# lighttransport/pbrlab

Hardware: AMD Instinct MI355X
Metric: Msamples/s (paths x spp / s), 1920x1080 Cornell-box-Suzanne render (higher is better)
Workload: dtype f32

## Files before the change

### pbrlab_amd/csrc/bvh_build.cpp

```cpp
#include <math.h>
#include <stdlib.h>
#include <string.h>

#include <algorithm>
#include <atomic>
#include <deque>
#include <functional>
#include <future>
#include <limits>
#include <thread>

#include "host_scene.h"
#include "qquant.h"

namespace pb {
namespace {

#ifndef PB_SAH_BINS
#define PB_SAH_BINS 48
#endif
constexpr int kBins = PB_SAH_BINS;
#ifndef PB_SAH_SWEEP
#define PB_SAH_SWEEP 256
#endif
#ifndef PB_MAX_LEAF_CURVES
#define PB_MAX_LEAF_CURVES PB_MAX_LEAF
#endif
constexpr float kTraversalCost = 1.0f;
constexpr float kPrimCost = 1.5f;

struct Box {
  float lo[3], hi[3];
  void reset() {
    for (int a = 0; a < 3; a++) lo[a] = std::numeric_limits<float>::infinity(), hi[a] = -lo[a];
  }
  void grow(const float* l, const float* h) {
    for (int a = 0; a < 3; a++) {
      lo[a] = std::min(lo[a], l[a]);
      hi[a] = std::max(hi[a], h[a]);
    }
  }
  void grow(const Box& b) { grow(b.lo, b.hi); }
  float area() const {
    float dx = hi[0] - lo[0], dy = hi[1] - lo[1], dz = hi[2] - lo[2];
    if (!(dx >= 0 && dy >= 0 && dz >= 0)) return 0.f;
    return 2.f * (dx * dy + dy * dz + dz * dx);
  }
};

struct TNode {
  Box box;
  int32_t left = -1, right = -1;
  uint32_t first = 0, count = 0;
  uint8_t kind = 0;
  uint32_t depth = 1;
};

struct Builder {
// ... 82 lines not shown
        }
        float rarea[kBins];
        uint32_t rcnt[kBins];
        Box acc;
        acc.reset();
        uint32_t n = 0;
        for (int k = kBins - 1; k > 0; k--) {
          acc.grow(bb[k]);
          n += bc[k];
          rarea[k] = acc.area();
          rcnt[k] = n;
        }
        acc.reset();
        n = 0;
        for (int k = 0; k < kBins - 1; k++) {
          acc.grow(bb[k]);
          n += bc[k];
          if (n == 0 || rcnt[k + 1] == 0) continue;
          float cost = acc.area() * (float)n + rarea[k + 1] * (float)rcnt[k + 1];
          if (cost < best_cost) best_cost = cost, best_axis = a, best_bin = k;
        }
      }
      if (best_axis >= 0) {
        float scale = (float)kBins / (cbox.hi[best_axis] - cbox.lo[best_axis]);
        float base = cbox.lo[best_axis];
        mid = (uint32_t)(std::partition(order.begin() + first, order.begin() + first + count,
                                        [&](uint32_t g) {
                                          int k = std::min(kBins - 1, std::max(0, (int)((cen[3 * g + best_axis] - base) * scale)));
                                          return k <= best_bin;
                                        }) -
                         order.begin());
      }
      if (mid == first || mid == first + count) {
        int a = 0;
        for (int c = 1; c < 3; c++)
          if (cbox.hi[c] - cbox.lo[c] > cbox.hi[a] - cbox.lo[a]) a = c;
        mid = first + count / 2;
        std::nth_element(order.begin() + first, order.begin() + mid, order.begin() + first + count,
                         [&](uint32_t x, uint32_t y) { return cen[3 * x + a] < cen[3 * y + a] || (cen[3 * x + a] == cen[3 * y + a] && x < y); });
      }
    }
    int32_t l = build(pool, first, mid - first, depth + 1);
    int32_t r = build(pool, mid, first + count - mid, depth + 1);
    pool.nodes[id].left = l;
    pool.nodes[id].right = r;
    return id;
  }
};

uint32_t leaf_ref(const TNode& n) {
  return kLeafBit | (n.kind ? kCurveBit : 0u) | (n.first << 3) | (n.count - 1u);
}

}

void build_bvh(const std::vector<float>& lo, const std::vector<float>& hi, const std::vector<uint8_t>& kinds,
               FlatBvh* out) {
  out->nodes.clear();
  out->slot_gid.clear();
  out->depth = 0;
  uint32_t n = (uint32_t)kinds.size();
  if (n == 0) return;
  Builder b;
  b.lo = lo.data(), b.hi = hi.data(), b.kinds = kinds.data();
  b.cen.resize(3 * (size_t)n);
  b.order.resize(n);
  for (uint32_t g = 0; g < n; g++) {
    for (int a = 0; a < 3; a++) b.cen[3 * g + a] = 0.5f * (lo[3 * g + a] + hi[3 * g + a]);
    b.order[g] = g;
  }
  Builder::Pool pool;
  pool.nodes.reserve(2 * (size_t)n / 2 + 16);
  int32_t root = b.build(pool, 0, n, 1);

  const std::vector<TNode>& T = pool.nodes;
  const float kNaN3[3] = {std::numeric_limits<float>::quiet_NaN(), std::numeric_limits<float>::quiet_NaN(),
                          std::numeric_limits<float>::quiet_NaN()};
  std::vector<BvhNode>& N = out->nodes;
  uint32_t depth = 0;
  if (T[root].left < 0) {
    BvhNode nd;
    memset(&nd, 0, sizeof(nd));
    nd.set_box(0, T[root].box.lo, T[root].box.hi);
    nd.set_box(1, kNaN3, kNaN3);
    nd.c0 = leaf_ref(T[root]);
    nd.c1 = kEmptyChild;
    N.push_back(nd);
    depth = 1;
  } else {
    struct Item {
      int32_t t;
      uint32_t out;
    };
    std::deque<Item> work;
    N.emplace_back();
    work.push_back({root, 0});
    while (!work.empty()) {
      Item it;
      if (N.size() < (size_t)kTopNodes) it = work.front(), work.pop_front();
      else it = work.back(), work.pop_back();
      const TNode& t = T[it.t];
      depth = std::max(depth, t.depth);
      BvhNode nd;
      memset(&nd, 0, sizeof(nd));
      const TNode &l = T[t.left], &r = T[t.right];
      nd.set_box(0, l.box.lo, l.box.hi);
      nd.set_box(1, r.box.lo, r.box.hi);
      if (l.left < 0) {
        nd.c0 = leaf_ref(l);
      } else {
        nd.c0 = (uint32_t)N.size();
        N.emplace_back();
        work.push_back({t.left, nd.c0});
      }
      if (r.left < 0) {
        nd.c1 = leaf_ref(r);
      } else {
        nd.c1 = (uint32_t)N.size();
        N.emplace_back();
        work.push_back({t.right, nd.c1});
      }
      N[it.out] = nd;
    }
  }
  out->slot_gid = b.order;
  out->depth = depth;
}


uint32_t qtree_stack_need(const std::vector<QNode>& N) {
  if (N.empty()) return 0;
  std::vector<uint32_t> need(N.size(), 0);
  std::vector<uint8_t> state(N.size(), 0);
  std::vector<uint32_t> todo{0u};
  while (!todo.empty()) {
    const uint32_t i = todo.back();
    const QNode& nd = N[i];
    if (state[i] == 0) {
      state[i] = 1;
      for (int k = 0; k < 4; k++)
        if (!(nd.c[k] & kLeafBit) && nd.c[k] < N.size() && state[nd.c[k]] == 0) todo.push_back(nd.c[k]);
      continue;
    }
    todo.pop_back();
    if (state[i] == 2) continue;
    state[i] = 2;
    uint32_t nc = 0, deepest = 0;
    for (int k = 0; k < 4; k++) {
      if (nd.c[k] == kEmptyChild) continue;
      nc++;
      if (!(nd.c[k] & kLeafBit) && nd.c[k] < N.size()) deepest = std::max(deepest, need[nd.c[k]]);
    }
    need[i] = (nc ? nc - 1u : 0u) + deepest;
  }
  return need[0];
}

uint32_t build_qtree(const std::vector<BvhNode>& N2, const std::function<uint32_t(uint32_t)>& map_leaf, std::vector<QNode>* out) {
  out->clear();
  if (N2.empty()) return 0;
  struct V {
    float lo[3], hi[3];
    int32_t l = -1, r = -1;
    uint32_t ref = 0;
    uint32_t prims = 0;
  };
  std::vector<V> T;
  T.reserve(N2.size() * 2 + 1);
  {
    struct Todo {
      uint32_t node2;
      int32_t v;
    };
    std::vector<Todo> todo;
    T.emplace_back();
    todo.push_back({0u, 0});
    while (!todo.empty()) {
      const Todo t = todo.back();
      todo.pop_back();
      const BvhNode& b = N2[t.node2];
      int32_t kids[2] = {-1, -1};
      int nk = 0;
      for (int k = 0; k < 2; k++) {
        const uint32_t ref = k ? b.c1 : b.c0;
        if (ref == kEmptyChild) continue;
        const int32_t v = (int32_t)T.size();
        T.emplace_back();
        for (int a = 0; a < 3; a++) T[v].lo[a] = b.lo[a][k], T[v].hi[a] = b.hi[a][k];
        kids[nk++] = v;
        if (ref & kLeafBit) T[v].ref = map_leaf(ref), T[v].prims = (ref & 7u) + 1u;
        else todo.push_back({ref, v});
      }
      if (nk == 2) T[t.v].l = kids[0], T[t.v].r = kids[1];
      else if (nk == 1) T[t.v].l = kids[0], T[t.v].r = -1;
    }
    for (int a = 0; a < 3; a++) {
      T[0].lo[a] = std::numeric_limits<float>::infinity(), T[0].hi[a] = -T[0].lo[a];
      for (int32_t k : {T[0].l, T[0].r})
        if (k >= 0) T[0].lo[a] = std::min(T[0].lo[a], T[k].lo[a]), T[0].hi[a] = std::max(T[0].hi[a], T[k].hi[a]);
    }
  }
  auto area = [](const V& v) {
    const float dx = v.hi[0] - v.lo[0], dy = v.hi[1] - v.lo[1], dz = v.hi[2] - v.lo[2];
    const float a = dx * dy + dy * dz + dz * dx;
    return a >= 0.f && std::isfinite(a) ? (double)a : 0.0;
  };
  constexpr double kCostNode = 1.0, kCostPrim = 1.0;
  const size_t nv = T.size();
  std::vector<double> below(nv, 0.0);
  std::vector<int32_t> choice(nv * 4, -1);
  auto qarea = [&](const V& u, const V& v) {
    double e[3];
    for (int a = 0; a < 3; a++) {
      const double ext = (double)v.hi[a] - (double)v.lo[a];
      const double st = std::max(ext / 253.0, 1e-37);
      const double ql = floor(((double)u.lo[a] - (double)v.lo[a]) / st), qh = ceil(((double)u.hi[a] - (double)v.lo[a]) / st);
      e[a] = std::max(qh - ql, 0.0) * st;
    }
    const double a = e[0] * e[1] + e[1] * e[2] + e[2] * e[0];
    return std::isfinite(a) ? a : 0.0;
  };
  for (size_t vi = nv; vi-- > 0;) {
    const V& v = T[vi];
    if (v.l < 0) continue;
    if (v.r < 0) {
      choice[vi * 4] = v.l;
      below[vi] = T[v.l].l < 0 ? area(T[v.l]) * kCostPrim * T[v.l].prims : area(T[v.l]) * kCostNode + below[v.l];
      continue;
    }
    int32_t fronts[16][4];
    int sizes[16], nf = 0;
    fronts[0][0] = v.l, fronts[0][1] = v.r, sizes[0] = 2, nf = 1;
    for (int i = 0; i < nf && nf < 16; i++) {
      if (sizes[i] >= 4) continue;
      for (int m = 0; m < sizes[i] && nf < 16; m++) {
        const V& u = T[fronts[i][m]];
        if (u.l < 0 || u.r < 0) continue;
        int32_t g[4];
        int n = 0;
        for (int j = 0; j < sizes[i]; j++) {
          if (j == m) g[n++] = u.l, g[n++] = u.r;
          else g[n++] = fronts[i][j];
        }
        std::sort(g, g + n);
        bool dup = false;
        for (int q = 0; q < nf && !dup; q++) dup = sizes[q] == n && std::equal(g, g + n, fronts[q]);
        if (dup) continue;
        std::copy(g, g + n, fronts[nf]), sizes[nf] = n, nf++;
      }
    }
    double best = 1e300;
    int bi = 0;
    for (int i = 0; i < nf; i++) {
      double c = 0.0;
      for (int m = 0; m < sizes[i]; m++) {
        const V& u = T[fronts[i][m]];
        c += u.l < 0 ? qarea(u, v) * kCostPrim * u.prims : qarea(u, v) * kCostNode + below[fronts[i][m]];
      }
      if (c < best) best = c, bi = i;
    }
    below[vi] = best;
    for (int m = 0; m < sizes[bi]; m++) choice[vi * 4 + m] = fronts[bi][m];
  }
  struct Item {
    int32_t v;
    uint32_t out;
  };
  std::deque<Item> work;
  out->emplace_back();
  work.push_back({0, 0u});
  while (!work.empty()) {
    Item it;
    if (out->size() < (size_t)kTopNodes) it = work.front(), work.pop_front();
    else it = work.back(), work.pop_back();
    int32_t fr[4];
    int n = 0;
    if (T[it.v].l < 0) {
      fr[n++] = it.v;
    } else {
      for (int m = 0; m < 4; m++)
        if (choice[(size_t)it.v * 4 + m] >= 0) fr[n++] = choice[(size_t)it.v * 4 + m];
    }
    QBox c[4];
    for (int i = 0; i < n; i++)
      for (int a = 0; a < 3; a++) c[i].lo[a] = T[fr[i]].lo[a], c[i].hi[a] = T[fr[i]].hi[a];
    QNode nd;
    if (n == 0 || !quantise_node(c, n, &nd)) {
      out->clear();
      return 0;
    }
    for (int i = 0; i < 4; i++) nd.c[i] = kEmptyChild;
    for (int i = 0; i < n; i++) {
      const V& u = T[fr[i]];
      if (u.l < 0) {
        nd.c[i] = u.ref;
      } else {
        const uint32_t id = (uint32_t)out->size();
        out->emplace_back();
        nd.c[i] = id;
        work.push_back({fr[i], id});
      }
    }
    (*out)[it.out] = nd;
  }
  return qtree_stack_need(*out);
}

void build_qlayout(const FlatBvh& bvh, const std::vector<float4>& slots, const std::vector<uint8_t>& kinds, QLayout* out) {
  static_assert(kMaxLeaf <= 2, "a leaf of the binary tree becomes one TriPair / one curve record");
  *out = QLayout();
  std::vector<float4>&qtri = out->tri, &qpts = out->pts;
  std::vector<uint32_t>& qhit = out->hit;
  const float4 zero = make_float4(0.f, 0.f, 0.f, 0.f);
  auto code = [&](uint32_t k) { return k | __builtin_bit_cast(uint32_t, slots[4 * (size_t)k + 2].w); };
  const bool tri_pairs = std::all_of(kinds.begin(), kinds.end(), [](uint8_t kd) { return kd == 0; });
  auto tri_leaf = [&](uint32_t first, uint32_t count) -> uint32_t {
// ... 113 lines not shown
```

### pbrlab_amd/csrc/commit.cpp

```cpp
#include <math.h>
#include <string.h>

#include <chrono>
#include <limits>
#include <numeric>

#include "scene_impl.h"

using namespace pb;

static_assert(sizeof(LightRec) == 80, "light record layout");

static V3 mesh_vertex(const HostMesh& m, uint32_t prim, int k) {
  const float* p = m.vertices.data() + (size_t)m.vid[prim * 3 + k] * 4;
  return V3(p[0], p[1], p[2]);
}
static V3 xf_point(const float* m, V3 v) {
  return V3(m[0] * v.x + m[4] * v.y + m[8] * v.z + m[12], m[1] * v.x + m[5] * v.y + m[9] * v.z + m[13],
            m[2] * v.x + m[6] * v.y + m[10] * v.z + m[14]);
}
static V3 world_vertex(const HostInstance& in, const HostMesh& m, uint32_t prim, int k) {
  const V3 v = mesh_vertex(m, prim, k);
  return in.identity ? v : xf_point(in.xf, v);
}
// ... 270 lines not shown
  sl[2].w = __builtin_bit_cast(float, route);
  sr.instance_id = pr.instance_id, sr.geom_id = pr.geom_id, sr.prim_id = pr.prim_id;
  return PBRHIP_OK;
}
static std::vector<BvhNode> light_boxes(const std::vector<LightHead>& heads, const std::vector<LightRec>& lrecs) {
  std::vector<BvhNode> boxes((heads.size() + 1) / 2);
  for (size_t l = 0; l < heads.size(); l++) {
    float lo3[3] = {INFINITY, INFINITY, INFINITY}, hi3[3] = {-INFINITY, -INFINITY, -INFINITY};
    for (uint32_t f = heads[l].first; f < heads[l].first + heads[l].count; f++)
      for (const float* p : {lrecs[f].p0, lrecs[f].p1, lrecs[f].p2})
        for (int a = 0; a < 3; a++) lo3[a] = std::min(lo3[a], p[a]), hi3[a] = std::max(hi3[a], p[a]);
    BvhNode& nd = boxes[l / 2];
    if (l % 2 == 0) memset(&nd, 0, sizeof(nd)), nd.set_box(1, lo3, hi3);
    nd.set_box(int(l % 2), lo3, hi3);
  }
  return boxes;
}

static double ms_since(std::chrono::steady_clock::time_point t) {
  return std::chrono::duration<double, std::milli>(std::chrono::steady_clock::now() - t).count();
}

struct CommitStage {
  std::vector<PrimRef> prims;
  std::vector<float> lo, hi, lprim_cdf;
  std::vector<uint8_t> kinds;
  FlatBvh bvh;
  std::vector<float4> slots;
  std::vector<ShadeRec> shade;
  std::vector<Material> mats;
  QLayout q;
  std::vector<LightRec> lrecs;
  std::vector<BvhNode> lboxes;
  std::vector<SssEntry> walk_entries;
};

static void stage_lights(pbrhip_scene* s, CommitStage* cs) {
  for (uint32_t i = 0; i < s->instances.size(); i++) register_lights(s, i);
  commit_lights(s);
  light_records(s, &s->light_heads, &cs->lrecs, &cs->lprim_cdf);
  cs->lboxes = light_boxes(s->light_heads, cs->lrecs);
  s->num_lrecs = (uint32_t)cs->lrecs.size();
  s->lights_transformed = std::any_of(s->lights.begin(), s->lights.end(), [&](const HostLight& L) { return !s->instances[L.instance_id].identity; });
}
static int upload_lights(pbrhip_scene* s, const CommitStage& cs) {
  HIPCHK(s->d_light_cdf.upload(s->light_cdf, s->stream));
  HIPCHK(s->d_heads.upload(s->light_heads, s->stream));
  HIPCHK(s->d_lprim_cdf.upload(cs.lprim_cdf, s->stream));
  HIPCHK(s->d_lrecs.upload(cs.lrecs, s->stream));
  HIPCHK(s->d_light_boxes.upload(cs.lboxes, s->stream));
  return PBRHIP_OK;
}

static int build_binary_tree(pbrhip_scene* s, int builder, CommitStage* cs) {
  FlatBvh& bvh = cs->bvh;
  const uint32_t np = (uint32_t)cs->prims.size();
  s->bvh_built_on_gpu = false;
  if ((builder == PBRHIP_BVH_GPU_LBVH || builder == PBRHIP_BVH_GPU_LBVH_WIDE) && np > 0) {
    HIPCHK(s->tree.reserve_nodes(TreeBufs::lbvh_nodes(np), np));
    HIPCHK(build_bvh_gpu(s->stream, cs->lo, cs->hi, cs->kinds, s->tree.d_nodes.p, &bvh.slot_gid, &bvh.depth));
    s->bvh_built_on_gpu = bvh.depth <= (uint32_t)kStackDepth;
    if (!s->bvh_built_on_gpu) {
      fprintf(stderr, "pbrhip: GPU-built BVH is %u deep (stack %d): building on the host instead\n", bvh.depth, kStackDepth);
      bvh = FlatBvh();
    }
  }
  if (!s->bvh_built_on_gpu) build_bvh(cs->lo, cs->hi, cs->kinds, &bvh);
  if (bvh.depth > (uint32_t)kStackDepth)
    return fail(PBRHIP_EOVERFLOW, "BVH depth %u exceeds the traversal stack (%d)", bvh.depth, kStackDepth);
  s->bvh_depth = bvh.depth;
  if (!s->bvh_built_on_gpu) {
    HIPCHK(s->tree.reserve_nodes((uint32_t)bvh.nodes.size(), (uint32_t)bvh.slot_gid.size()));
    if (!bvh.nodes.empty()) HIPCHK(hipMemcpyAsync(s->tree.d_nodes.p, bvh.nodes.data(), bvh.nodes.size() * sizeof(BvhNode), hipMemcpyHostToDevice, s->stream));
  }
  return PBRHIP_OK;
}

static int stage_slots_and_materials(pbrhip_scene* s, CommitStage* cs) {
  const uint32_t ns = (uint32_t)cs->bvh.slot_gid.size();
  if (ns > kHitSlotMask) return fail(PBRHIP_EINVAL, "%u traversal primitives: at most %u are supported", ns, kHitSlotMask);
  cs->slots.resize(4 * (size_t)ns), cs->shade.resize(ns);
  for (uint32_t k = 0; k < ns; k++)
    if (int rc = slot_and_shade(s, cs->prims[cs->bvh.slot_gid[k]], cs->bvh.slot_gid[k], s->light_heads, &cs->slots[4 * (size_t)k], cs->shade[k])) return rc;
  std::vector<Material>& mats = cs->mats;
  mats.resize(s->materials.size());
  s->has_hair = s->has_sss = s->has_textured = false;
  for (size_t i = 0; i < mats.size(); i++) {
    const HostMaterial& hm = s->materials[i];
    if (hm.kind == kMatPrincipled)
      for (uint32_t t : {hm.pr.base_color_tex_id, hm.pr.subsurface_color_tex_id})
        if (t != kNone && t >= s->tex_descs.size()) return fail(PBRHIP_EINVAL, "material %zu: texture id %u out of range", i, t);
    mats[i] = make_material(s->materials[i]);
    if (mats[i].textured) s->has_sss = s->has_textured = true;
    s->has_hair = s->has_hair || mats[i].kind == kMatHair;
    s->has_sss = s->has_sss || (mats[i].kind == kMatPrincipled && mats[i].bsdf.enable_subsurface);
  }
  return PBRHIP_OK;
}

static int build_wide_tree(pbrhip_scene* s, const Knobs& k, int builder, CommitStage* cs) {
  TreeBufs& t = s->tree;
  QLayout& q = cs->q;
  s->wide_built_on_gpu = false;
  if (!s->bvh_built_on_gpu && t.num_nodes && k.wide) {
    build_qlayout(cs->bvh, cs->slots, cs->kinds, &q);
    if (k.debug) fprintf(stderr, "pbrhip: commit: curve leaves of the Q tree (counted over the collapse's visits): %zu of one piece, %zu of two pieces\n", q.leaves_one, q.leaves_pair);
  }
  if (s->bvh_built_on_gpu && builder == PBRHIP_BVH_GPU_LBVH_WIDE && k.wide) {
    const bool tri_pairs = all_triangles(cs->kinds);
    QCollapse qc;
    HIPCHK(hipStreamSynchronize(s->stream));
    const auto t_start = std::chrono::steady_clock::now();
    HIPCHK(collapse_qtree_gpu(s->stream, t.d_nodes.p, t.num_slots, t.slots(), tri_pairs, [&](auto... a) { return t.alloc_wide(a...); }, &qc));
    const double ms_collapse = ms_since(t_start);
    const char* why = !qc.fits ? "a record index overflows its reference" : (!qc.quantised ? "a node cannot be quantised" : nullptr);
    if (!why) {
      q.nodes.resize(qc.nodes);
      HIPCHK(hipMemcpyAsync(q.nodes.data(), t.d_wide.p, (size_t)qc.nodes * sizeof(QNode), hipMemcpyDeviceToHost, s->stream));
      HIPCHK(hipStreamSynchronize(s->stream));
      q.stack_need = qtree_stack_need(q.nodes);
// ... 14 lines not shown
  s->wide_stack_need = q.nodes.empty() ? 0u : q.stack_need;
  return PBRHIP_OK;
}

static void accumulate_instance_bounds(std::vector<float>& ilo, std::vector<float>& ihi, size_t inst, const float* lo, const float* hi) {
  for (size_t a = 0; a < 3; a++) ilo[3 * inst + a] = std::min(ilo[3 * inst + a], lo[a]), ihi[3 * inst + a] = std::max(ihi[3 * inst + a], hi[a]);
}

static int update_walk_entries(pbrhip_scene* s, const Knobs& k, bool want, const std::vector<float>& ilo, const std::vector<float>& ihi, CommitStage* cs, double* ms) {
  cs->walk_entries.clear();
  if (want && !cs->q.nodes.empty()) {
    const auto t_entries = std::chrono::steady_clock::now();
    cs->walk_entries = build_sss_entries(cs->q.nodes, ilo, ihi, std::min(k.sss_foreign, kSssMaxForeign));
    if (ms) *ms = ms_since(t_entries);
  }
  s->num_walk_entries = (uint32_t)cs->walk_entries.size();
  if (cs->walk_entries.empty()) s->d_sss_entries.release();
  else HIPCHK(s->d_sss_entries.upload(cs->walk_entries, s->stream));
  return PBRHIP_OK;
}

void pb::bind_dscene(pbrhip_scene* s) {
  DScene& d = s->dscene;
  const TreeBufs& t = s->tree;
  d.nodes = t.d_nodes.p, d.slots = t.slots(), d.num_nodes = t.num_nodes, d.num_slots = t.num_slots;
  d.top_nodes = s->bvh_built_on_gpu ? 0u : std::min<uint32_t>(t.num_nodes, (uint32_t)kTopNodes);
  d.wide = t.wide_nodes ? t.d_wide.p : nullptr, d.q_hitcode = t.wide_nodes ? t.d_qhit.p : nullptr, d.wide_nodes = t.wide_nodes;
  d.q_tri0 = (uint32_t)t.tri0(), d.q_pt0 = (uint32_t)t.pt0();
  d.wide_top_nodes = std::min<uint32_t>(t.wide_nodes, (uint32_t)kTopNodes);
  d.shade = s->d_shade.p, d.num_curves = s->num_curves;
  d.materials = s->d_materials.p, d.num_materials = (uint32_t)s->materials.size();
  d.light_cdf = s->d_light_cdf.p, d.light_heads = s->d_heads.p, d.num_lights = (uint32_t)s->lights.size();
  d.lprim_cdf = s->d_lprim_cdf.p, d.lrecs = s->d_lrecs.p, d.num_lrecs = s->num_lrecs;
  d.light_boxes = s->d_light_boxes.p, d.lights_transformed = s->lights_transformed ? 1u : 0u;
  d.tex_pixels = s->d_tex_pixels.p, d.textures = s->d_tex_descs.p, d.num_textures = (uint32_t)s->tex_descs.size();
  d.sss_entries = s->num_walk_entries ? s->d_sss_entries.p : nullptr, d.num_sss_entries = s->num_walk_entries;
}

extern "C" int pbrhip_scene_commit(pbrhip_scene* s) {
  return guarded([&]() -> int {
  if (!s) return fail(PBRHIP_EINVAL, "scene is NULL");
  const Knobs k = read_knobs();
  HIPCHK(hipSetDevice(s->device));
  const int builder = k.bvh >= 0 ? k.bvh : s->bvh_builder;
  CommitStage cs;
  s->committed = false;
  stage_lights(s, &cs);
  if (int rc = flatten_prims(s, &cs.prims)) return rc;
  const uint32_t np = (uint32_t)cs.prims.size();
  if (np >= (1u << 27)) return fail(PBRHIP_EUNSUPPORTED, "too many primitives (%u)", np);
  prim_boxes(s, cs.prims, &cs.lo, &cs.hi, &cs.kinds);
  scene_bounds(s);
  s->num_curves = (uint32_t)(cs.kinds.size() - std::count(cs.kinds.begin(), cs.kinds.end(), 0));
  if (int rc = build_binary_tree(s, builder, &cs)) return rc;
  if (int rc = stage_slots_and_materials(s, &cs)) return rc;
  const TreeBufs& t = s->tree;
  if (t.num_slots) HIPCHK(hipMemcpyAsync(t.slots(), cs.slots.data(), (size_t)t.num_slots * 64, hipMemcpyHostToDevice, s->stream));
  if (int rc = build_wide_tree(s, k, builder, &cs)) return rc;
  s->inst_lo.assign(3 * s->instances.size(), INFINITY), s->inst_hi.assign(3 * s->instances.size(), -INFINITY);
  for (size_t g = 0; g < cs.prims.size(); g++) accumulate_instance_bounds(s->inst_lo, s->inst_hi, cs.prims[g].instance_id, &cs.lo[3 * g], &cs.hi[3 * g]);
  double ms_entries = -1.0;
  if (int rc = update_walk_entries(s, k, k.sss_entry, s->inst_lo, s->inst_hi, &cs, &ms_entries)) return rc;
  if (k.debug) {
    if (ms_entries >= 0.0) fprintf(stderr, "pbrhip: commit: random walks' entries over %zu wide nodes: %.2f ms\n", cs.q.nodes.size(), ms_entries);
    for (size_t i = 0; i < cs.walk_entries.size(); i++)
      if (cs.walk_entries[i].entry) fprintf(stderr, "pbrhip: commit: instance %zu: random walks start at Q node %u with %u foreign references\n", i, cs.walk_entries[i].entry, cs.walk_entries[i].nforeign);
    fprintf(stderr, "pbrhip: commit: %u binary nodes, %zu wide nodes, %zu slots, %zu triangle leaves + %zu points in the Q tree\n", t.num_nodes, (size_t)t.wide_nodes, (size_t)t.num_slots, t.tri_words / kTriPairWords, t.points);
  }
  HIPCHK(s->d_shade.upload(cs.shade, s->stream));
  HIPCHK(s->d_materials.upload(cs.mats, s->stream));
  if (int rc = upload_lights(s, cs)) return rc;
  HIPCHK(s->d_tex_pixels.upload(s->tex_pixels, s->stream));
  HIPCHK(s->d_tex_descs.upload(s->tex_descs, s->stream));
  HIPCHK(hipStreamSynchronize(s->stream));
  bind_dscene(s);
  s->slot_gid = std::move(cs.bvh.slot_gid);
  s->rf_plan.release();
  s->dirty_inst.assign(s->instances.size(), 0), s->stale = false;
  s->committed = true;
  return PBRHIP_OK;
  });
}

int pb::update_material(pbrhip_scene* s, uint32_t id, const HostMaterial& hm) {
  if (id >= s->materials.size()) return fail(PBRHIP_EINVAL, "material id %u out of range", id);
  if (s->materials[id].kind != hm.kind) return fail(PBRHIP_EINVAL, "material %u is of the other kind", id);
  if (s->committed && hm.kind == kMatPrincipled)
    for (uint32_t t : {hm.pr.base_color_tex_id, hm.pr.subsurface_color_tex_id})
      if (t != kNone && t >= s->tex_descs.size()) return fail(PBRHIP_EINVAL, "texture id %u out of range", t);
  if (s->committed) {
    HIPCHK(hipSetDevice(s->device));
    const Material m = make_material(hm);
    HIPCHK(hipMemcpyAsync(s->d_materials.p + id, &m, sizeof(m), hipMemcpyHostToDevice, s->stream));
    HIPCHK(hipStreamSynchronize(s->stream));
    s->has_sss = s->has_sss || (m.kind == kMatPrincipled && (m.bsdf.enable_subsurface || m.textured));
    s->has_textured = s->has_textured || (m.kind == kMatPrincipled && m.textured);
  }
  s->materials[id] = hm;
  return PBRHIP_OK;
}

extern "C" int pbrhip_scene_refit(pbrhip_scene* s) {
  return guarded([&]() -> int {
  if (!s) return fail(PBRHIP_EINVAL, "scene is NULL");
  if (s->replica) return fail(PBRHIP_ESTATE, "scene_refit: a replica holds no geometry (refit the source scene and replicate it again)");
  if (!s->committed) return fail(PBRHIP_ESTATE, "scene not committed");
  if (!s->stale) return PBRHIP_OK;
// ... 75 lines not shown
```

### pbrlab_amd/csrc/host_scene.h

```cpp
#pragma once

#include <stdint.h>

#include <functional>
#include <string>
#include <vector>

#include "dshade.h"

namespace pb {

struct HostMesh {
  int kind = 0;
  std::vector<float> vertices, normals, texcoords;
  std::vector<uint32_t> vid, nid, tid, mat;
  uint32_t nfaces = 0;
  std::vector<float> cverts;
  std::vector<uint32_t> cidx, cmat;
  uint32_t num_prims() const { return kind == 0 ? nfaces : (uint32_t)cidx.size(); }
};

struct HostAreaLight {
  std::vector<uint32_t> light_param_ids;
  std::vector<float> choose_prob, cdf, area_pdf;
  float intensity_sum = 0.f;
  uint32_t global_id = kNone;
};

struct HostInstance {
  uint32_t local_scene = 0;
  float xf[16];
  bool identity = true;
  std::vector<std::vector<uint32_t>> material_ids, light_ids;
  std::vector<int> has_area_light;
  std::vector<HostAreaLight> area_lights;
};

struct HostMaterial {
  uint32_t kind = kMatPrincipled;
  PrincipledParam pr;
  HairParam hr;
};

struct HostLight {
  float choose_prob = 0.f;
  uint32_t instance_id = 0, geom_id = 0;
};

struct PrimRef {
  uint32_t instance_id, geom_id, prim_id, kind, sub;
};

struct FlatBvh {
  std::vector<BvhNode> nodes;
  std::vector<uint32_t> slot_gid;
  uint32_t depth = 0;
};

void build_bvh(const std::vector<float>& lo, const std::vector<float>& hi, const std::vector<uint8_t>& kinds,
               FlatBvh* out);

uint32_t build_qtree(const std::vector<BvhNode>& nodes, const std::function<uint32_t(uint32_t)>& map_leaf, std::vector<QNode>* out);

struct QLayout {
  std::vector<QNode> nodes;
  std::vector<float4> tri, pts;
  std::vector<uint32_t> hit;
  uint32_t stack_need = 0;
  size_t leaves_one = 0, leaves_pair = 0;
};
void build_qlayout(const FlatBvh& bvh, const std::vector<float4>& slots, const std::vector<uint8_t>& kinds, QLayout* out);

std::vector<SssEntry> build_sss_entries(const std::vector<QNode>& wide, const std::vector<float>& ilo, const std::vector<float>& ihi,
                                        uint32_t max_foreign);

hipError_t build_bvh_gpu(hipStream_t st, const std::vector<float>& lo, const std::vector<float>& hi,
                         const std::vector<uint8_t>& kinds, BvhNode* nodes_out, std::vector<uint32_t>* order_out,
                         uint32_t* depth_out);

struct QCollapse {
  uint32_t nodes = 0;
  size_t tri_words = 0, pts = 0;
  uint32_t levels = 0;
  double alloc_ms = 0.0;
  bool fits = false;
  bool quantised = false;
};
hipError_t collapse_qtree_gpu(hipStream_t st, const BvhNode* d_nodes, uint32_t n, const float4* d_slots, bool tri_pairs,
                              const std::function<hipError_t(size_t, size_t, float4**, uint32_t**)>& alloc, QCollapse* out);
struct RefitPlan {
  uint32_t* d_list = nullptr;
  float4* d_qbox = nullptr;
  float4* d_bbox = nullptr;
  uint32_t* d_cnt = nullptr;
  std::vector<uint32_t> bin_off, q_off;
  bool built = false;
  RefitPlan() = default;
  RefitPlan(const RefitPlan&) = delete;
  RefitPlan& operator=(const RefitPlan&) = delete;
  ~RefitPlan() { release(); }
  void release();
};
struct RefitTree {
  BvhNode* nodes = nullptr;
  uint32_t nb = 0, ns = 0;
  QNode* q = nullptr;
  uint32_t nq = 0;
  float4* tri = nullptr;
  size_t tri_words = 0;
  bool tri_pairs = false;
  float4* pts = nullptr;
  const uint32_t* hit = nullptr;
  size_t npts = 0;
// ... 12 lines not shown
```

### pbrlab_amd/csrc/knobs.h

```cpp
#pragma once

#include <stdint.h>
#include <optional>

#ifndef PB_QUAD_RAYS
#define PB_QUAD_RAYS 0u
#endif

namespace pb {

struct Knobs {
  int bvh = -1;
  bool wide = true;
  bool sss_entry = true;
  uint32_t sss_foreign = 3;
  bool debug = false;
  uint32_t pixel_tile = 8;
  bool patch_shuffle = true;
  uint32_t pass_run = 0;
  const char* groups = nullptr;
  std::optional<uint32_t> tail_paths;
  std::optional<uint32_t> streams;
  uint32_t window = 8;
  uint32_t bulk_div = 0;
  uint32_t pipe_depth = 2;
  uint32_t pipe_depth_small = 8;
  double pipe_stop = 2.0;
  bool trace_sched = false;
  const char* wave_log = nullptr;
  bool pv_stats = false;
  uint32_t susp_turns = 24;
  uint32_t shadow_first = 1;
  bool first_direct = true;
  bool direct = true;
  bool sss_walk = true;
  bool wide_walk = true;
  uint32_t rays_per_wave = 4;
  uint32_t trace_blocks = 0;
  bool small_caps = true;
  uint32_t small_blocks = 0, small_rays = 0;
  uint32_t quad_rays = PB_QUAD_RAYS;
  bool quad = false;
  bool simple_traversal = false;
};

Knobs read_knobs();

}
```

### pbrlab_amd/csrc/pbrhip.cpp

```cpp
#include <hip/hip_runtime.h>
#include <math.h>
#include <stdarg.h>
#include <stdio.h>
#include <stdlib.h>
#include <string.h>

#include <algorithm>
#include <chrono>
#include <memory>
#include <string>
#include <thread>
#include <vector>

#include "env_tables.h"
#include "feature_kernels.h"
#include "scene_impl.h"

using namespace pb;

static_assert(sizeof(pbrhip_principled_param) == sizeof(PrincipledParam), "param layout");
static_assert(sizeof(pbrhip_hair_param) == sizeof(HairParam), "param layout");

static thread_local std::string g_err;
static int g_device = 0;

int pb::fail(int code, const char* fmt, ...) {
  char buf[512];
  va_list ap;
  va_start(ap, fmt);
  vsnprintf(buf, sizeof(buf), fmt, ap);
  va_end(ap);
  g_err = buf;
  return code;
}
int pb::current_device() { return g_device; }

extern "C" const char* pbrhip_last_error(void) { return g_err.c_str(); }
extern "C" uint32_t pbrhip_abi_version(void) { return PBRHIP_ABI_VERSION; }
extern "C" uint32_t pbrhip_math_mode(void) { return pb::kMathMode; }
extern "C" size_t pbrhip_sizeof_render_stats(void) { return sizeof(pbrhip_render_stats); }

extern "C" int pbrhip_device_count(int* count) {
  if (!count) return fail(PBRHIP_EINVAL, "count is NULL");
  int n = 0;
  hipError_t e = hipGetDeviceCount(&n);
  if (e != hipSuccess) {
    *count = 0;
    return fail(PBRHIP_ENODEVICE, "hipGetDeviceCount: %s", hipGetErrorString(e));
  }
  *count = n;
  return PBRHIP_OK;
}
extern "C" int pbrhip_set_device(int device) {
  int n = 0;
  int rc = pbrhip_device_count(&n);
  if (rc) return rc;
  if (device < 0 || device >= n) return fail(PBRHIP_EINVAL, "device %d out of range (%d devices)", device, n);
  g_device = device;
  return PBRHIP_OK;
}

Knobs pb::read_knobs() {
  auto env = [](const char* name) -> const char* { return getenv(name); };
  auto u32 = [&](const char* name, uint32_t dflt) { const char* e = env(name); return e ? (uint32_t)strtoul(e, nullptr, 10) : dflt; };
  auto not_zero = [&](const char* name) { const char* e = env(name); return !(e && atoi(e) == 0); };
  Knobs k;
  if (const char* e = env("PBRHIP_BVH")) k.bvh = strcmp(e, "gpu-wide") == 0 ? PBRHIP_BVH_GPU_LBVH_WIDE : (strcmp(e, "gpu") == 0 ? PBRHIP_BVH_GPU_LBVH : PBRHIP_BVH_HOST_SAH);
  k.wide = not_zero("PBRHIP_WIDE");
  k.sss_entry = u32("PBRHIP_SSS_ENTRY", 1u) != 0u;
  k.sss_foreign = u32("PBRHIP_SSS_FOREIGN", 3u);
  k.debug = env("PBRHIP_DEBUG") != nullptr;
  k.pixel_tile = u32("PBRHIP_PIXEL_TILE", 8u);
  k.patch_shuffle = u32("PBRHIP_PATCH_SHUFFLE", 1u) != 0u;
  if (const char* e = env("PBRHIP_PASS_RUN")) k.pass_run = std::max(1u, (uint32_t)strtoul(e, nullptr, 10));
  k.groups = env("PBRHIP_GROUPS");
  if (const char* e = env("PBRHIP_TAIL_PATHS")) k.tail_paths = (uint32_t)strtoul(e, nullptr, 10);
  if (const char* e = env("PBRHIP_STREAMS")) k.streams = (uint32_t)atoi(e);
  k.window = std::max(1u, u32("PBRHIP_WINDOW", k.groups ? 1u : (uint32_t)kMaxGroups));
  k.bulk_div = u32("PBRHIP_BULK_DIV", 0u);
  k.pipe_depth = std::min(std::max(1u, u32("PBRHIP_PIPE_DEPTH", 2u)), kRingSlots - 1u);
  k.pipe_depth_small = std::min(std::max(1u, u32("PBRHIP_PIPE_DEPTH_SMALL", 8u)), kRingSlots - 1u);
  if (const char* e = env("PBRHIP_PIPE_STOP")) k.pipe_stop = atof(e);
  k.trace_sched = env("PBRHIP_TRACE_SCHED") != nullptr;
  k.wave_log = env("PBRHIP_WAVE_LOG");
  k.pv_stats = env("PBRHIP_PV_STATS") != nullptr;
  k.susp_turns = u32("PBRHIP_SUSP_TURNS", 24u);
  k.shadow_first = u32("PBRHIP_SHADOW_FIRST", 1u);
  k.first_direct = u32("PBRHIP_FIRST_DIRECT", 1u) != 0u;
  k.direct = u32("PBRHIP_DIRECT", 1u) != 0u;
  k.sss_walk = u32("PBRHIP_SSS_WALK", 1u) != 0u;
  k.wide_walk = not_zero("PBRHIP_WIDE_WALK");
  k.rays_per_wave = u32("PBRHIP_RAYS_PER_WAVE", 4u);
  k.trace_blocks = u32("PBRHIP_TRACE_BLOCKS", 0u);
  if (const char* e = env("PBRHIP_TRACE_BLOCKS_SMALL")) {
    char* end = nullptr;
    k.small_caps = false;
    k.small_blocks = (uint32_t)strtoul(e, &end, 10);
    k.small_rays = (end && *end == ',') ? (uint32_t)strtoul(end + 1, nullptr, 10) : 0u;
  }
  k.quad_rays = u32("PBRHIP_QUAD_RAYS", PB_QUAD_RAYS);
  if (const char* e = env("PBRHIP_QUAD")) k.quad = e[0] == '1';
  k.simple_traversal = env("PBRHIP_SIMPLE_TRAVERSAL") != nullptr;
  return k;
}

extern "C" int pbrhip_scene_create(pbrhip_scene** out) {
  return guarded([&]() -> int {
  if (!out) return fail(PBRHIP_EINVAL, "out is NULL");
  int n = 0;
  int rc = pbrhip_device_count(&n);
  if (rc) return rc;
  if (n <= 0) return fail(PBRHIP_ENODEVICE, "no HIP device available: libpbrhip has no CPU fallback");
  HIPCHK(hipSetDevice(g_device));
  std::unique_ptr<pbrhip_scene> s(new pbrhip_scene());
  s->device = g_device;
  HIPCHK(hipStreamCreateWithFlags(&s->stream, hipStreamNonBlocking));
  HIPCHK(hipHostMalloc((void**)&s->h_counts, sizeof(uint32_t) * kCntNum * kMaxGroups, hipHostMallocDefault));
  HIPCHK(hipHostMalloc((void**)&s->h_ring, sizeof(uint32_t) * 4 * kRingSlots * kMaxGroups, hipHostMallocDefault));
  memset(s->h_ring, 0, sizeof(uint32_t) * 4 * kRingSlots * kMaxGroups);
  HIPCHK(hipHostGetDevicePointer((void**)&s->d_ring, s->h_ring, 0));
  memset(&s->dscene, 0, sizeof(s->dscene));
// ... 1301 lines not shown
```

Baseline: 2959.

## Add greedy subtree re-insertion pass to optimize host SAH BVH

After the top-down SAH build, a post-pass takes the largest-area nodes, unlinks each one and re-inserts it at the position found by a branch-and-bound search that minimizes the added surface area. Each pass is kept only if it lowers a cost, either the quantized 4-wide collapse cost (reusing the collapse DP, refactored into shared helpers with incremental dirty re-evaluation) or the total inner area, and only if traversal stack depth still fits. The goal is better tree quality and fewer traversal steps per ray, in exchange for more host build time at commit. It is enabled by default for triangle-only scenes.

```diff
diff --git a/pbrlab_amd/csrc/bvh_build.cpp b/pbrlab_amd/csrc/bvh_build.cpp
--- a/pbrlab_amd/csrc/bvh_build.cpp
+++ b/pbrlab_amd/csrc/bvh_build.cpp
@@ -4,6 +4,7 @@
 
 #include <algorithm>
 #include <atomic>
+#include <chrono>
 #include <deque>
 #include <functional>
 #include <future>
@@ -192,13 +193,313 @@
   return kLeafBit | (n.kind ? kCurveBit : 0u) | (n.first << 3) | (n.count - 1u);
 }
 
+struct QV {
+  float lo[3], hi[3];
+  int32_t l = -1, r = -1;
+  uint32_t ref = 0;
+  uint32_t prims = 0;
+};
+
+void qv_of_nodes(const std::vector<BvhNode>& N2, const std::function<uint32_t(uint32_t)>& map_leaf, std::vector<QV>* out) {
+  std::vector<QV>& T = *out;
+  T.clear();
+  T.reserve(N2.size() * 2 + 1);
+  struct Todo {
+    uint32_t node2;
+    int32_t v;
+  };
+  std::vector<Todo> todo;
+  T.emplace_back();
+  todo.push_back({0u, 0});
+  while (!todo.empty()) {
+    const Todo t = todo.back();
+    todo.pop_back();
+    const BvhNode& b = N2[t.node2];
+    int32_t kids[2] = {-1, -1};
+    int nk = 0;
+    for (int k = 0; k < 2; k++) {
+      const uint32_t ref = k ? b.c1 : b.c0;
+      if (ref == kEmptyChild) continue;
+      const int32_t v = (int32_t)T.size();
+      T.emplace_back();
+      for (int a = 0; a < 3; a++) T[v].lo[a] = b.lo[a][k], T[v].hi[a] = b.hi[a][k];
+      kids[nk++] = v;
+      if (ref & kLeafBit) T[v].ref = map_leaf(ref), T[v].prims = (ref & 7u) + 1u;
+      else todo.push_back({ref, v});
+    }
+    if (nk == 2) T[t.v].l = kids[0], T[t.v].r = kids[1];
+    else if (nk == 1) T[t.v].l = kids[0], T[t.v].r = -1;
+  }
+  for (int a = 0; a < 3; a++) {
+    T[0].lo[a] = std::numeric_limits<float>::infinity(), T[0].hi[a] = -T[0].lo[a];
+    for (int32_t k : {T[0].l, T[0].r})
+      if (k >= 0) T[0].lo[a] = std::min(T[0].lo[a], T[k].lo[a]), T[0].hi[a] = std::max(T[0].hi[a], T[k].hi[a]);
+  }
+}
+
+void qdp_vertex(const std::vector<QV>& T, size_t vi, std::vector<double>& below, std::vector<int32_t>& choice) {
+  using V = QV;
+  auto area = [](const V& v) {
+    const float dx = v.hi[0] - v.lo[0], dy = v.hi[1] - v.lo[1], dz = v.hi[2] - v.lo[2];
+    const float a = dx * dy + dy * dz + dz * dx;
+    return a >= 0.f && std::isfinite(a) ? (double)a : 0.0;
+  };
+  constexpr double kCostNode = 1.0, kCostPrim = 1.0;
+  auto qarea = [&](const V& u, const V& v) {
+    double e[3];
+    for (int a = 0; a < 3; a++) {
+      const double ext = (double)v.hi[a] - (double)v.lo[a];
+      const double st = std::max(ext / 253.0, 1e-37);
+      const double ql = floor(((double)u.lo[a] - (double)v.lo[a]) / st), qh = ceil(((double)u.hi[a] - (double)v.lo[a]) / st);
+      e[a] = std::max(qh - ql, 0.0) * st;
+    }
+    const double a = e[0] * e[1] + e[1] * e[2] + e[2] * e[0];
+    return std::isfinite(a) ? a : 0.0;
+  };
+  const V& v = T[vi];
+  for (int m = 0; m < 4; m++) choice[vi * 4 + m] = -1;
+  below[vi] = 0.0;
+  if (v.l < 0) return;
+  if (v.r < 0) {
+    choice[vi * 4] = v.l;
+    below[vi] = T[v.l].l < 0 ? area(T[v.l]) * kCostPrim * T[v.l].prims : area(T[v.l]) * kCostNode + below[v.l];
+    return;
+  }
+  int32_t fronts[16][4];
+  int sizes[16], nf = 0;
+  fronts[0][0] = v.l, fronts[0][1] = v.r, sizes[0] = 2, nf = 1;
+  for (int i = 0; i < nf && nf < 16; i++) {
+    if (sizes[i] >= 4) continue;
+    for (int m = 0; m < sizes[i] && nf < 16; m++) {
+      const V& u = T[fronts[i][m]];
+      if (u.l < 0 || u.r < 0) continue;
+      int32_t g[4];
+      int n = 0;
+      for (int j = 0; j < sizes[i]; j++) {
+        if (j == m) g[n++] = u.l, g[n++] = u.r;
+        else g[n++] = fronts[i][j];
+      }
+      std::sort(g, g + n);
+      bool dup = false;
+      for (int q = 0; q < nf && !dup; q++) dup = sizes[q] == n && std::equal(g, g + n, fronts[q]);
+      if (dup) continue;
+      std::copy(g, g + n, fronts[nf]), sizes[nf] = n, nf++;
+    }
+  }
+  int32_t term_of[16];
+  double term[16];
+  int nt = 0;
+  auto member = [&](int32_t ui) {
+    for (int k = 0; k < nt; k++)
+      if (term_of[k] == ui) return term[k];
+    const V& u = T[ui];
+    term_of[nt] = ui, term[nt] = u.l < 0 ? qarea(u, v) * kCostPrim * u.prims : qarea(u, v) * kCostNode + below[ui];
+    return term[nt++];
+  };
+  double best = 1e300;
+  int bi = 0;
+  for (int i = 0; i < nf; i++) {
+    double c = 0.0;
+    for (int m = 0; m < sizes[i]; m++) c += member(fronts[i][m]);
+    if (c < best) best = c, bi = i;
+  }
+  below[vi] = best;
+  for (int m = 0; m < sizes[bi]; m++) choice[vi * 4 + m] = fronts[bi][m];
+}
+
+uint32_t qdp_need(const std::vector<QV>& T, size_t vi, const std::vector<int32_t>& choice, const std::vector<uint32_t>& need) {
+  uint32_t nc = 0, deepest = 0;
+  for (int m = 0; m < 4; m++) {
+    const int32_t u = choice[vi * 4 + m];
+    if (u < 0) continue;
+    nc++;
+    if (T[u].l >= 0) deepest = std::max(deepest, need[u]);
+  }
+  return (nc ? nc - 1u : 0u) + deepest;
+}
+
+
+struct Reinserter {
+  std::vector<TNode>& T;
+  int32_t root;
+  const BvhBuildOptions& opt;
+  std::vector<int32_t> parent;
+  std::vector<QV> qv;
+  std::vector<double> below;
+  std::vector<int32_t> choice;
+  std::vector<uint32_t> need;
+  std::vector<uint8_t> dirty;
+  struct Move {
+    int32_t n, sibling;
+  };
+  std::vector<Move> log;
+
+  static Box unite(const Box& a, const Box& b) {
+    Box u = a;
+    u.grow(b);
+    return u;
+  }
+  void replace_child(int32_t g, int32_t from, int32_t to) { (T[g].left == from ? T[g].left : T[g].right) = to; }
+  void refit_up(int32_t i) {
+    for (; i >= 0; i = parent[i]) {
+      const Box b = unite(T[T[i].left].box, T[T[i].right].box);
+      if (memcmp(&b, &T[i].box, sizeof(Box)) == 0) break;
+      T[i].box = b;
+    }
+  }
+  void mark_up(int32_t i) {
+    if (dirty.empty()) return;
+    for (; i >= 0; i = parent[i]) dirty[i] = 1;
+  }
+  int32_t unlink(int32_t n) {
+    const int32_t p = parent[n], g = parent[p], s = T[p].left == n ? T[p].right : T[p].left;
+    parent[s] = g;
+    if (g < 0) root = s;
+    else replace_child(g, p, s), refit_up(g);
+    return p;
+  }
+  void link(int32_t p, int32_t n, int32_t x) {
+    const int32_t g = parent[x];
+    (T[p].left == n ? T[p].right : T[p].left) = x;
+    parent[x] = p, parent[p] = g;
+    T[p].box = unite(T[x].box, T[n].box);
+    if (g < 0) root = p;
+    else replace_child(g, x, p), refit_up(g);
+  }
+
+  uint32_t pass() {
+    std::vector<std::pair<float, int32_t>> cand;
+    cand.reserve(T.size());
+    for (int32_t i = 0; i < (int32_t)T.size(); i++)
+      if (i != root && parent[i] != root) cand.push_back({T[i].box.area(), i});
+    const size_t K = std::min<size_t>(opt.reinsert_top, cand.size());
+    auto larger = [](const std::pair<float, int32_t>& a, const std::pair<float, int32_t>& b) {
+      return a.first > b.first || (a.first == b.first && a.second < b.second);
+    };
+    if (K < cand.size()) std::nth_element(cand.begin(), cand.begin() + (ptrdiff_t)K, cand.end(), larger);
+    std::sort(cand.begin(), cand.begin() + (ptrdiff_t)K, larger);
+    using Entry = std::pair<double, int32_t>;
+    std::vector<Entry> heap;
+    uint32_t moves = 0;
+    for (size_t c = 0; c < K; c++) {
+      const int32_t n = cand[c].second;
+      if (n == root || parent[n] == root) continue;
+      const int32_t s = T[parent[n]].left == n ? T[parent[n]].right : T[parent[n]].left;
+      const int32_t p = unlink(n);
+      const Box nb = T[n].box;
+      const double an = nb.area();
+      double best = unite(T[s].box, nb).area();
+      for (int32_t a = parent[s]; a >= 0; a = parent[a]) best += (double)unite(T[a].box, nb).area() - (double)T[a].box.area();
+      int32_t bx = s;
+      heap.clear();
+      heap.push_back({0.0, root});
+      while (!heap.empty()) {
+        std::pop_heap(heap.begin(), heap.end(), std::greater<Entry>());
+        const Entry e = heap.back();
+        heap.pop_back();
+        if (!(e.first + an < best)) break;
+        const int32_t x = e.second;
+        const double total = e.first + (double)unite(T[x].box, nb).area();
+        if (total < best) best = total, bx = x;
+        const double grown = total - (double)T[x].box.area();
+        if (T[x].left >= 0 && grown + an < best) {
+          heap.push_back({grown, T[x].left}), std::push_heap(heap.begin(), heap.end(), std::greater<Entry>());
+          heap.push_back({grown, T[x].right}), std::push_heap(heap.begin(), heap.end(), std::greater<Entry>());
+        }
+      }
+      const int32_t g = parent[s];
+      link(p, n, bx);
+      if (bx == s) continue;
+      mark_up(g), mark_up(p);
+      log.push_back({n, s});
+      moves++;
+    }
+    return moves;
+  }
+  void undo_pass() {
+    for (size_t i = log.size(); i-- > 0;) link(unlink(log[i].n), log[i].n, log[i].sibling);
+    log.clear();
+  }
+
+  double evaluate() {
+    std::vector<int32_t> todo{root}, pre;
+    while (!todo.empty()) {
+      const int32_t i = todo.back();
+      todo.pop_back();
+      if (!dirty[i]) continue;
+      pre.push_back(i);
+      if (T[i].left >= 0) todo.push_back(T[i].left), todo.push_back(T[i].right);
+    }
+    for (size_t k = pre.size(); k-- > 0;) {
+      const int32_t i = pre[k];
+      const TNode& t = T[i];
+      QV& q = qv[i];
+      for (int a = 0; a < 3; a++) q.lo[a] = BvhNode::widen_lo(t.box.lo[a]), q.hi[a] = BvhNode::widen_hi(t.box.hi[a]);
+      q.l = t.left, q.r = t.right, q.prims = t.left < 0 ? t.count : 0u;
+      qdp_vertex(qv, (size_t)i, below, choice);
+      need[i] = qdp_need(qv, (size_t)i, choice, need);
+      dirty[i] = 0;
+    }
+    return below[root];
+  }
+  double inner_area() const {
+    double sum = 0.0;
+    for (const TNode& t : T)
+      if (t.left >= 0) sum += (double)t.box.area();
+    return sum;
+  }
+  uint32_t set_depths() {
+    uint32_t deepest = 0;
+    std::vector<int32_t> todo{root};
+    T[root].depth = 1;
+    while (!todo.empty()) {
+      const int32_t i = todo.back();
+      todo.pop_back();
+      if (T[i].left < 0) continue;
+      deepest = std::max(deepest, T[i].depth);
+      T[T[i].left].depth = T[T[i].right].depth = T[i].depth + 1;
+      todo.push_back(T[i].left), todo.push_back(T[i].right);
+    }
+    return deepest;
+  }
+
+  void run(FlatBvh* out) {
+    if (T[root].left < 0) return;
+    parent.assign(T.size(), -1);
+    for (int32_t i = 0; i < (int32_t)T.size(); i++)
+      if (T[i].left >= 0) parent[T[i].left] = parent[T[i].right] = i;
+    bool by_q = opt.for_qtree;
+    double cost = 0.0;
+    if (by_q) {
+      qv.resize(T.size()), below.assign(T.size(), 0.0), choice.assign(T.size() * 4, -1), need.assign(T.size(), 0u), dirty.assign(T.size(), 1);
+      cost = evaluate();
+      by_q = need[root] <= (uint32_t)kStackDepth;
+      if (!by_q) dirty.clear();
+    }
+    if (!by_q) cost = inner_area();
+    out->reinsert_cost0 = out->reinsert_cost = cost;
+    for (uint32_t k = 0; k < opt.reinsert_passes; k++) {
+      const uint32_t moves = pass();
+      if (moves == 0) break;
+      const double c = by_q ? evaluate() : inner_area();
+      const bool fits = set_depths() <= (uint32_t)kStackDepth && (!by_q || need[root] <= (uint32_t)kStackDepth);
+      if (!(c < cost) || !fits) {
+        undo_pass();
+        break;
+      }
+      log.clear();
+      cost = c;
+      out->reinsert_cost = c, out->reinsert_passes++, out->reinsert_moves += moves;
+    }
+    set_depths();
+  }
+};
+
 }
 
 void build_bvh(const std::vector<float>& lo, const std::vector<float>& hi, const std::vector<uint8_t>& kinds,
-               FlatBvh* out) {
-  out->nodes.clear();
-  out->slot_gid.clear();
-  out->depth = 0;
+               FlatBvh* out, const BvhBuildOptions& opt) {
+  *out = FlatBvh();
   uint32_t n = (uint32_t)kinds.size();
   if (n == 0) return;
   Builder b;
@@ -211,7 +512,16 @@
   }
   Builder::Pool pool;
   pool.nodes.reserve(2 * (size_t)n / 2 + 16);
+  const auto t_build = std::chrono::steady_clock::now();
   int32_t root = b.build(pool, 0, n, 1);
+  const auto t_reinsert = std::chrono::steady_clock::now();
+  out->build_ms = std::chrono::duration<double, std::milli>(t_reinsert - t_build).count();
+  if (opt.reinsert_passes > 0 && opt.reinsert_top > 0 && std::all_of(kinds.begin(), kinds.end(), [](uint8_t kd) { return kd == 0; })) {
+    Reinserter re{pool.nodes, root, opt};
+    re.run(out);
+    root = re.root;
+    out->reinsert_ms = std::chrono::duration<double, std::milli>(std::chrono::steady_clock::now() - t_reinsert).count();
+  }
 
   const std::vector<TNode>& T = pool.nodes;
   const float kNaN3[3] = {std::numeric_limits<float>::quiet_NaN(), std::numeric_limits<float>::quiet_NaN(),
@@ -296,112 +606,33 @@
   return need[0];
 }
 
+double qtree_cost(const std::vector<BvhNode>& N2, uint32_t* stack_need) {
+  if (stack_need) *stack_need = 0;
+  if (N2.empty()) return 0.0;
+  std::vector<QV> T;
+  qv_of_nodes(N2, [](uint32_t ref) { return ref; }, &T);
+  const size_t nv = T.size();
+  std::vector<double> below(nv, 0.0);
+  std::vector<int32_t> choice(nv * 4, -1);
+  std::vector<uint32_t> need(nv, 0u);
+  for (size_t vi = nv; vi-- > 0;) {
+    qdp_vertex(T, vi, below, choice);
+    need[vi] = qdp_need(T, vi, choice, need);
+  }
+  if (stack_need) *stack_need = need[0];
+  return below[0];
+}
+
 uint32_t build_qtree(const std::vector<BvhNode>& N2, const std::function<uint32_t(uint32_t)>& map_leaf, std::vector<QNode>* out) {
   out->clear();
   if (N2.empty()) return 0;
-  struct V {
-    float lo[3], hi[3];
-    int32_t l = -1, r = -1;
-    uint32_t ref = 0;
-    uint32_t prims = 0;
-  };
+  using V = QV;
   std::vector<V> T;
-  T.reserve(N2.size() * 2 + 1);
-  {
-    struct Todo {
-      uint32_t node2;
-      int32_t v;
-    };
-    std::vector<Todo> todo;
-    T.emplace_back();
-    todo.push_back({0u, 0});
-    while (!todo.empty()) {
-      const Todo t = todo.back();
-      todo.pop_back();
-      const BvhNode& b = N2[t.node2];
-      int32_t kids[2] = {-1, -1};
-      int nk = 0;
-      for (int k = 0; k < 2; k++) {
-        const uint32_t ref = k ? b.c1 : b.c0;
-        if (ref == kEmptyChild) continue;
-        const int32_t v = (int32_t)T.size();
-        T.emplace_back();
-        for (int a = 0; a < 3; a++) T[v].lo[a] = b.lo[a][k], T[v].hi[a] = b.hi[a][k];
-        kids[nk++] = v;
-        if (ref & kLeafBit) T[v].ref = map_leaf(ref), T[v].prims = (ref & 7u) + 1u;
-        else todo.push_back({ref, v});
-      }
-      if (nk == 2) T[t.v].l = kids[0], T[t.v].r = kids[1];
-      else if (nk == 1) T[t.v].l = kids[0], T[t.v].r = -1;
-    }
-    for (int a = 0; a < 3; a++) {
-      T[0].lo[a] = std::numeric_limits<float>::infinity(), T[0].hi[a] = -T[0].lo[a];
-      for (int32_t k : {T[0].l, T[0].r})
-        if (k >= 0) T[0].lo[a] = std::min(T[0].lo[a], T[k].lo[a]), T[0].hi[a] = std::max(T[0].hi[a], T[k].hi[a]);
-    }
-  }
-  auto area = [](const V& v) {
-    const float dx = v.hi[0] - v.lo[0], dy = v.hi[1] - v.lo[1], dz = v.hi[2] - v.lo[2];
-    const float a = dx * dy + dy * dz + dz * dx;
-    return a >= 0.f && std::isfinite(a) ? (double)a : 0.0;
-  };
-  constexpr double kCostNode = 1.0, kCostPrim = 1.0;
+  qv_of_nodes(N2, map_leaf, &T);
   const size_t nv = T.size();
   std::vector<double> below(nv, 0.0);
   std::vector<int32_t> choice(nv * 4, -1);
-  auto qarea = [&](const V& u, const V& v) {
-    double e[3];
-    for (int a = 0; a < 3; a++) {
-      const double ext = (double)v.hi[a] - (double)v.lo[a];
-      const double st = std::max(ext / 253.0, 1e-37);
-      const double ql = floor(((double)u.lo[a] - (double)v.lo[a]) / st), qh = ceil(((double)u.hi[a] - (double)v.lo[a]) / st);
-      e[a] = std::max(qh - ql, 0.0) * st;
-    }
-    const double a = e[0] * e[1] + e[1] * e[2] + e[2] * e[0];
-    return std::isfinite(a) ? a : 0.0;
-  };
-  for (size_t vi = nv; vi-- > 0;) {
-    const V& v = T[vi];
-    if (v.l < 0) continue;
-    if (v.r < 0) {
-      choice[vi * 4] = v.l;
-      below[vi] = T[v.l].l < 0 ? area(T[v.l]) * kCostPrim * T[v.l].prims : area(T[v.l]) * kCostNode + below[v.l];
-      continue;
-    }
-    int32_t fronts[16][4];
-    int sizes[16], nf = 0;
-    fronts[0][0] = v.l, fronts[0][1] = v.r, sizes[0] = 2, nf = 1;
-    for (int i = 0; i < nf && nf < 16; i++) {
-      if (sizes[i] >= 4) continue;
-      for (int m = 0; m < sizes[i] && nf < 16; m++) {
-        const V& u = T[fronts[i][m]];
-        if (u.l < 0 || u.r < 0) continue;
-        int32_t g[4];
-        int n = 0;
-        for (int j = 0; j < sizes[i]; j++) {
-          if (j == m) g[n++] = u.l, g[n++] = u.r;
-          else g[n++] = fronts[i][j];
-        }
-        std::sort(g, g + n);
-        bool dup = false;
-        for (int q = 0; q < nf && !dup; q++) dup = sizes[q] == n && std::equal(g, g + n, fronts[q]);
-        if (dup) continue;
-        std::copy(g, g + n, fronts[nf]), sizes[nf] = n, nf++;
-      }
-    }
-    double best = 1e300;
-    int bi = 0;
-    for (int i = 0; i < nf; i++) {
-      double c = 0.0;
-      for (int m = 0; m < sizes[i]; m++) {
-        const V& u = T[fronts[i][m]];
-        c += u.l < 0 ? qarea(u, v) * kCostPrim * u.prims : qarea(u, v) * kCostNode + below[fronts[i][m]];
-      }
-      if (c < best) best = c, bi = i;
-    }
-    below[vi] = best;
-    for (int m = 0; m < sizes[bi]; m++) choice[vi * 4 + m] = fronts[bi][m];
-  }
+  for (size_t vi = nv; vi-- > 0;) qdp_vertex(T, vi, below, choice);
   struct Item {
     int32_t v;
     uint32_t out;
diff --git a/pbrlab_amd/csrc/commit.cpp b/pbrlab_amd/csrc/commit.cpp
--- a/pbrlab_amd/csrc/commit.cpp
+++ b/pbrlab_amd/csrc/commit.cpp
@@ -346,7 +346,7 @@
   return PBRHIP_OK;
 }
 
-static int build_binary_tree(pbrhip_scene* s, int builder, CommitStage* cs) {
+static int build_binary_tree(pbrhip_scene* s, const Knobs& k, int builder, CommitStage* cs) {
   FlatBvh& bvh = cs->bvh;
   const uint32_t np = (uint32_t)cs->prims.size();
   s->bvh_built_on_gpu = false;
@@ -359,7 +359,15 @@
       bvh = FlatBvh();
     }
   }
-  if (!s->bvh_built_on_gpu) build_bvh(cs->lo, cs->hi, cs->kinds, &bvh);
+  if (!s->bvh_built_on_gpu) {
+    BvhBuildOptions opt;
+    opt.reinsert_passes = k.bvh_reinsert ? kReinsertPasses : 0u, opt.reinsert_top = k.bvh_reinsert_top;
+    opt.for_qtree = k.wide;
+    build_bvh(cs->lo, cs->hi, cs->kinds, &bvh, opt);
+    if (k.debug)
+      fprintf(stderr, "pbrhip: commit: host BVH: top-down build %.2f ms; re-insertion %.2f ms: %u passes kept, %u subtrees moved, %s %.6g -> %.6g\n", bvh.build_ms,
+              bvh.reinsert_ms, bvh.reinsert_passes, bvh.reinsert_moves, k.wide ? "collapse cost" : "inner area", bvh.reinsert_cost0, bvh.reinsert_cost);
+  }
   if (bvh.depth > (uint32_t)kStackDepth)
     return fail(PBRHIP_EOVERFLOW, "BVH depth %u exceeds the traversal stack (%d)", bvh.depth, kStackDepth);
   s->bvh_depth = bvh.depth;
@@ -480,7 +488,7 @@
   prim_boxes(s, cs.prims, &cs.lo, &cs.hi, &cs.kinds);
   scene_bounds(s);
   s->num_curves = (uint32_t)(cs.kinds.size() - std::count(cs.kinds.begin(), cs.kinds.end(), 0));
-  if (int rc = build_binary_tree(s, builder, &cs)) return rc;
+  if (int rc = build_binary_tree(s, k, builder, &cs)) return rc;
   if (int rc = stage_slots_and_materials(s, &cs)) return rc;
   const TreeBufs& t = s->tree;
   if (t.num_slots) HIPCHK(hipMemcpyAsync(t.slots(), cs.slots.data(), (size_t)t.num_slots * 64, hipMemcpyHostToDevice, s->stream));
diff --git a/pbrlab_amd/csrc/host_scene.h b/pbrlab_amd/csrc/host_scene.h
--- a/pbrlab_amd/csrc/host_scene.h
+++ b/pbrlab_amd/csrc/host_scene.h
@@ -55,10 +55,22 @@
   std::vector<BvhNode> nodes;
   std::vector<uint32_t> slot_gid;
   uint32_t depth = 0;
+  uint32_t reinsert_passes = 0, reinsert_moves = 0;
+  double reinsert_cost0 = 0.0, reinsert_cost = 0.0;
+  double build_ms = 0.0, reinsert_ms = 0.0;
+};
+
+constexpr uint32_t kReinsertPasses = 4, kReinsertTop = 20000;
+struct BvhBuildOptions {
+  uint32_t reinsert_passes = 0;
+  uint32_t reinsert_top = kReinsertTop;
+  bool for_qtree = true;
 };
 
 void build_bvh(const std::vector<float>& lo, const std::vector<float>& hi, const std::vector<uint8_t>& kinds,
-               FlatBvh* out);
+               FlatBvh* out, const BvhBuildOptions& opt = BvhBuildOptions());
+
+double qtree_cost(const std::vector<BvhNode>& nodes, uint32_t* stack_need);
 
 uint32_t build_qtree(const std::vector<BvhNode>& nodes, const std::function<uint32_t(uint32_t)>& map_leaf, std::vector<QNode>* out);
 
diff --git a/pbrlab_amd/csrc/knobs.h b/pbrlab_amd/csrc/knobs.h
--- a/pbrlab_amd/csrc/knobs.h
+++ b/pbrlab_amd/csrc/knobs.h
@@ -12,6 +12,8 @@
 struct Knobs {
   int bvh = -1;
   bool wide = true;
+  bool bvh_reinsert = true;
+  uint32_t bvh_reinsert_top = 20000;
   bool sss_entry = true;
   uint32_t sss_foreign = 3;
   bool debug = false;
diff --git a/pbrlab_amd/csrc/pbrhip.cpp b/pbrlab_amd/csrc/pbrhip.cpp
--- a/pbrlab_amd/csrc/pbrhip.cpp
+++ b/pbrlab_amd/csrc/pbrhip.cpp
@@ -67,6 +67,8 @@
   Knobs k;
   if (const char* e = env("PBRHIP_BVH")) k.bvh = strcmp(e, "gpu-wide") == 0 ? PBRHIP_BVH_GPU_LBVH_WIDE : (strcmp(e, "gpu") == 0 ? PBRHIP_BVH_GPU_LBVH : PBRHIP_BVH_HOST_SAH);
   k.wide = not_zero("PBRHIP_WIDE");
+  k.bvh_reinsert = u32("PBRHIP_BVH_REINSERT", 1u) != 0u;
+  k.bvh_reinsert_top = u32("PBRHIP_BVH_REINSERT_TOP", kReinsertTop);
   k.sss_entry = u32("PBRHIP_SSS_ENTRY", 1u) != 0u;
   k.sss_foreign = u32("PBRHIP_SSS_FOREIGN", 3u);
   k.debug = env("PBRHIP_DEBUG") != nullptr;
```

Measured after the change: 3079, median of 6. 1.04x the previous value.
